# theteamatx/x-edr-trajectory-planning

Measured on AMD Instinct MI355X. Metric: time-optimal path timings/s (7-DOF, 2000 s-samples), 1/2/4/8 MI355X + %HBM roofline, higher is better.
Workload: dtype f64

## Files before the change

x-edr-trajectory-planning_amd/csrc/tpamd_capi.hip:

```cpp
#include "../../include/tpamd.h"

#include <hip/hip_runtime.h>

#include <algorithm>
#include <cmath>
#include <cstdio>
#include <cstdlib>
#include <cstring>
#include <mutex>
#include <new>
#include <vector>

#include "tpamd_kernels.h"
#include "tpamd_launch.h"
#include "tpamd_planner_set.h"
#include "tpamd_readout.h"
#include "tpamd_rescale.h"
#include "tpamd_buffer.h"
#include "tpamd_stop.h"
#include "tpamd_switch.h"
#include "tpamd_fit.h"
#include "tpamd_pose_fit.h"
#include "tpamd_sweep_joint.h"

// ... 181 lines not shown
  Lane lanes[kMaxLanes];
  hipEvent_t ev_fork = nullptr;
  bool in_lane = false;
  hipEvent_t front_wait = nullptr, front_record = nullptr;
  int phase = 0;
  std::vector<hipEvent_t> back_wait;
  int max_lanes = 4;
  int chain_fronts = 2;
  bool order_ragged = true;
  int k1_tpb = 0;
  int k1_tpb_ragged = 64;
  int front_delay_us = 10;
  std::vector<EventPair> events;
  std::vector<EventPair> pool;
  double acc_ms[KI_COUNT] = {};
  int acc_n[KI_COUNT] = {};
};

namespace {

size_t carve_workspace(char *base, int B, int N, int C, Workspace *ws) {
  Stage s(base);
  const size_t nb = (size_t)B, ns = (size_t)B * N;
  Workspace w{};
  w.ds = s.take<double>(nb);
  w.s_start = s.take<double>(nb);
  w.s_end = s.take<double>(nb);
  w.sd_start = s.take<double>(nb);
  w.sdd_start = s.take<double>(nb);
  w.t_start = s.take<double>(nb);
  w.delta = s.take<double>(nb);
  w.err_bits = s.take<uint32_t>(nb);
  w.lim = s.take<double>(nb * 2 * C);
  w.q12 = s.take<double>((ns + kTileSamples) * (C + 2));
  w.m0 = s.take<double>(ns);
  w.z0 = s.take<double>(ns);
  w.X0 = s.take<double>(ns);
  w.Y0 = s.take<double>(ns);
  w.Xz = s.take<double>(ns);
  w.Yz = s.take<double>(ns);
  w.at0 = s.take<uint8_t>(ns);
  w.fix_flag = s.take<uint8_t>(ns);
  w.fix_val = s.take<double>(ns);
  w.m = s.take<double>(ns);
  w.X = s.take<double>(ns);
  w.Y = s.take<double>(ns);
  w.type = s.take<uint8_t>(ns);
  w.sd2 = s.take<double>(ns);
  w.diag = s.take<long long>(nb * kDiagRow);
  w.order = s.take<int32_t>(nb);
  if (ws) *ws = w;
  return s.off;
}

int ensure_workspace(tpamd_engine *e, int B, int N, int C) {
  const size_t need = carve_workspace(nullptr, B, N, C, nullptr);
  if (need > e->ws_buf.bytes) {
    if (e->ws_buf.reserve(need)) return TPAMD_E_HIP;
#ifdef TPAMD_K1_STUDY
    HIPCHK(hipMemset(e->ws_buf.p, 0, need));
#endif
  }
  carve_workspace((char *)e->ws_buf.p, B, N, C, &e->ws);
  e->ws.keep_boundary = e->keep_boundary ? 1 : 0;
#ifdef TPAMD_K1_STUDY
  {
    static void *g_study = nullptr;
// ... 697 lines not shown
    return TPAMD_E_INVALID_ARGUMENT;
  return 0;
}

int cartesian_args(const tpamd_cartesian_batch *bt, const tpamd_cartesian_inputs *in,
                   const tpamd_path_outputs *out) {
  const int D = bt->num_dofs, N = bt->num_samples;
  if (D < 1 || D > 16 || N < 3 || N > 8192) return TPAMD_E_UNSUPPORTED;
  if (!in->ik_positions || !in->jacobians || !in->max_velocity || !in->max_acceleration ||
      !in->max_translational_velocity || !in->max_rotational_velocity || !in->path_start ||
      !in->delta || !in->sd_start || !in->time_start || !out->time || !out->s || !out->sd ||
      !out->sdd || !out->status)
    return TPAMD_E_INVALID_ARGUMENT;
  return 0;
}

int solve_cartesian(tpamd_engine *e, const tpamd_cartesian_batch *bt, const tpamd_cartesian_inputs *in,
                    const tpamd_path_outputs *out, void *hip_stream, const PlanParams *plan, int table_stride) {
  if (!e || !bt || !in || !out) return TPAMD_E_INVALID_ARGUMENT;
  const int B = bt->num_paths, D = bt->num_dofs, N = bt->num_samples;
  if (B <= 0) return B == 0 ? 0 : TPAMD_E_INVALID_ARGUMENT;
  if (int rc = cartesian_args(bt, in, out)) return rc;
  TPAMD_ON_DEVICE(e);
  hipStream_t st = (hipStream_t)hip_stream;
  const int C = 2 * D + 2;
  const int max_loops = bt->max_solver_loops > 0 ? bt->max_solver_loops : 0;
  const bool fused = (D == 6 || D == 7) && !e->force_generic;
  const int stride = plan ? table_stride : N;
  const int *first = plan ? plan->first : nullptr;
  const unsigned gb = (unsigned)((B + 127) / 128);
  PlanParams pp{};
  if (plan) {
    pp = *plan;
    pp.rec_stride = fused ? C + 2 : 2 * D + 2;
  }
  SlotGuard slot_guard(e, st);
  int rc = ensure_workspace(e, B, N, C);
  if (rc) return rc;
  e->last_B = B; e->last_N = N; e->last_time = out->time;
  e->ws.ns = nullptr;
  e->ws.order = nullptr;
  e->ws.amax = in->max_acceleration;
  {
    Timer t(e, st, KI_SETUP);
    hipLaunchKernelGGL(k_setup_cartesian, dim3((B + 127) / 128), dim3(128), 0, st, B, N, D,
                       bt->constraint_safety, in->max_velocity, in->max_acceleration,
                       in->max_translational_velocity, in->max_rotational_velocity,
                       in->path_start, in->delta, in->sd_start, in->sdd_start, in->time_start,
                       e->ws);
    if (plan) hipLaunchKernelGGL(k_plan_mark_skipped, dim3(gb), dim3(128), 0, st, pp, e->ws);
  }
  if (fused) {
    const Workspace &ws = e->ws;
    {
      Timer t(e, st, KI_SAMPLE_LP);
      const int tpb = 256;
      const size_t lds = (2 * (size_t)C + (2 * (size_t)D + 2) * tpb) * 8;
      const dim3 grid((N + tpb - 1) / tpb, B);
      if (D == 6)
        hipLaunchKernelGGL((k_cartesian_lp<1, 6>), grid, dim3(tpb), lds, st, N, in->ik_positions,
                           in->jacobians, ws, stride, first);
      else
        hipLaunchKernelGGL((k_cartesian_lp<1, 7>), grid, dim3(tpb), lds, st, N, in->ik_positions,
                           in->jacobians, ws, stride, first);
      if (plan) hipLaunchKernelGGL(k_plan_project, dim3(gb), dim3(128), 0, st, pp, ws);
    }
    JointSource src;
// ... 2994 lines not shown
```

x-edr-trajectory-planning_amd/csrc/tpamd_kernels.h:

```cpp
#pragma once

#include "tpamd_device.h"
#include "tpamd_cartesian_window.h"
#include "tpamd_quat.h"

namespace tpamd {

constexpr int kDiagExt = 16;
constexpr int kDiagRow = 64 + 2 * kDiagExt;

struct Workspace {
  double *ds, *s_start, *s_end, *sd_start, *sdd_start, *t_start, *delta;
  uint32_t *err_bits;
  const int32_t *ns;
  const double *amax;
  const int32_t *order;
  double *lim;
  double *q12;
  double *m0, *z0, *X0, *Y0, *Xz, *Yz;
  uint8_t *at0;
  uint8_t *fix_flag;
  double *fix_val;
  double *m, *X, *Y;
  uint8_t *type;
// ... 19 lines not shown
  const int tid = threadIdx.x;
  const int shift = (N > 8192) ? 5 : 3;
  hist[tid] = 0;
  __syncthreads();
  for (int b = tid; b < B; b += 1024) {
    const int n = min(max(ns[b], 0), N);
    atomicAdd(&hist[min((N - n) >> shift, kOrderBins - 1)], 1);
  }
  __syncthreads();
  scan[tid] = hist[tid];
  __syncthreads();
  for (int off = 1; off < kOrderBins; off <<= 1) {
    const int v = (tid >= off) ? scan[tid - off] : 0;
    __syncthreads();
    scan[tid] += v;
    __syncthreads();
  }
  hist[tid] = scan[tid] - hist[tid];
  __syncthreads();
  for (int b = tid; b < B; b += 1024) {
    const int n = min(max(ns[b], 0), N);
    order[atomicAdd(&hist[min((N - n) >> shift, kOrderBins - 1)], 1)] = b;
  }
}

struct JointSource {
  const double *q12;
  const double *lim;
  int D;
  int E = 0;
  __device__ __forceinline__ int rows() const { return 2 * D + E; }
  __device__ __forceinline__ int b_only_from() const { return D; }
  static constexpr bool kJoint = true;
  __device__ __forceinline__ int stride() const { return 2 * D + E + 2; }
  __device__ __forceinline__ JointRowsAt at(int b, int N, int idx) const {
    JointRowsAt r;
    r.q12 = q12 + ((size_t)b * N + idx) * stride();
    r.lim_lo = lim + (size_t)b * 2 * rows();
    r.lim_hi = r.lim_lo + rows();
    r.D = D;
    r.E = E;
    return r;
  }
};

struct GenericSource {
  const double *A, *B, *LO, *HI;
  int C;
  __device__ __forceinline__ int rows() const { return C; }
  __device__ __forceinline__ int b_only_from() const { return -1; }
  static constexpr bool kJoint = false;
  __device__ __forceinline__ GlobalRowsAt at(int b, int N, int idx) const {
    const size_t o = ((size_t)b * N + idx) * C;
    GlobalRowsAt r;
    r.A = A + o; r.B = B + o; r.LO = LO + o; r.HI = HI + o;
    return r;
  }
};

static __global__ void k_setup_joint(int B, int N, int D, double safety, const double *vmax,
                              const double *amax, const double *path_start,
                              const double *delta, const double *sd_start,
                              const double *sdd_start, const double *t_start, Workspace ws) {
  const int b = blockIdx.x * blockDim.x + threadIdx.x;
  if (b >= B) return;
  const int C = 2 * D;
  double *lo = ws.lim + (size_t)b * 2 * C, *hi = lo + C;
// ... 140 lines not shown
  if (!live) {
  } else if (parameter < kend + delta) {
    double u = parameter;
    if (u < k0) u = k0;
    if (kend < u) u = kend;
    const int span = knot_span_deg2(s_knots, Kb, u);
    double ders[3][3];
    basis_ders_deg2(s_knots, span, u, ders);
    const double *p0 = s_cp + (size_t)(span - 2) * D, *p1 = p0 + D, *p2 = p1 + D;
#pragma unroll
    for (int d = 0; d < D; d++) {
      double v0 = 0.0, v1 = 0.0, v2 = 0.0;
      v0 += ders[0][0] * p0[d]; v0 += ders[0][1] * p1[d]; v0 += ders[0][2] * p2[d];
      v1 += ders[1][0] * p0[d]; v1 += ders[1][1] * p1[d]; v1 += ders[1][2] * p2[d];
      v2 += ders[2][0] * p0[d]; v2 += ders[2][1] * p1[d]; v2 += ders[2][2] * p2[d];
      if (q_out) q_out[o * D + d] = v0;
      Q1[d * TPB] = v1;
      Q2[d * TPB] = v2;
      if (DT) { q1r[d] = v1; q2r[d] = v2; }
    }
  } else {
    const double *pl = s_cp + (size_t)(Pb - 1) * D;
#pragma unroll
    for (int d = 0; d < D; d++) {
      if (q_out) q_out[o * D + d] = pl[d];
      Q1[d * TPB] = 0.0;
      Q2[d * TPB] = 0.0;
      if (DT) { q1r[d] = 0.0; q2r[d] = 0.0; }
    }
  }
  __syncthreads();
  {
    const int nvalid = min(TPB, Nb - i0);
    double2 *recs = reinterpret_cast<double2 *>(ws.q12 + ((size_t)b * N + i0) * (C + 2));
    const int pairs = D + 1;
    for (int c = tid; c < nvalid * pairs; c += TPB) {
      const int sm = c / pairs, pr = c - sm * pairs;
      recs[c] = (pr < D) ? make_double2(s_Q1[pr * TPB + sm], s_Q2[pr * TPB + sm]) : make_double2(0.0, 0.0);
    }
  }
  if (!live) return;
  LdsRowsJoint r;
  r.Q1 = Q1; r.Q2 = Q2; r.lim_lo = s_lo; r.lim_hi = s_hi; r.stride = TPB; r.D = D;
  if (DT) {
    double sd2max, sddmax, sd2zero, x0, y0;
    lp_find_max_sd2<WORDS, LdsRowsJoint, DT, 2 * DT>(r, C, &sd2max, &sddmax, &sd2zero, D,
                                                     q1r, q2r);
    find_sdd_both_joint_screened<(DT ? DT : 1)>(q1r, q2r, Q1, Q2, TPB, s_hi, sd2max, &x0, &y0);
    ws.m0[o] = sd2max;
    ws.z0[o] = sd2zero;
    ws.X0[o] = x0;
    ws.Y0[o] = y0;
    ws.at0[o] = fabs(sd2max - sd2zero) < kTiny;
  } else {
    boundary_point<WORDS, true>(r, C, o, ws);
  }
#ifdef TPAMD_K1_STUDY
  __syncthreads();
  if (threadIdx.x == 0) {
    unsigned long long t;
    asm volatile("s_memrealtime %0\n\ts_waitcnt lgkmcnt(0)" : "=s"(t)::"memory");
    reinterpret_cast<unsigned long long *>(ws.diag)[2 * (blockIdx.y * gridDim.x + blockIdx.x) + 1] = t;
  }
#endif
}

#ifdef TPAMD_K1_STUDY
#define TPAMD_K1_STUDY_REGS __attribute__((amdgpu_waves_per_eu(5, 5)))
#else
#define TPAMD_K1_STUDY_REGS
#endif
// ... 72 lines not shown
  double ders[3][3];
  basis_ders_deg2(s_knots, span, parameter, ders);
  const double b0 = ders[0][0], b1 = ders[0][1], b2 = ders[0][2];
  const double *t0 = s_t + 3 * (span - 2);
  for (int d = 0; d < 3; d++) {
    double v = 0.0;
    v += b0 * t0[d]; v += b1 * t0[3 + d]; v += b2 * t0[6 + d];
    out[d] = v;
  }
  const double cum1 = b2, cum0 = cum1 + b1;
  const double *r0 = s_r + 4 * (span - 2);
  const Quat p0 = {r0[0], r0[1], r0[2], r0[3]}, p1 = {r0[4], r0[5], r0[6], r0[7]},
             p2 = {r0[8], r0[9], r0[10], r0[11]};
  Quat q = p0;
  q = quat_mul(q, quat_power(quat_mul(quat_inverse(p0), p1), cum0));
  q = quat_mul(q, quat_power(quat_mul(quat_inverse(p1), p2), cum1));
  quat_normalize_positive_real(q);
  out[3] = q.w; out[4] = q.x; out[5] = q.y; out[6] = q.z;
}

static __global__ void k_cartesian_rows(int N, int D, double safety, const double *q_g,
                                 const double *J_g, const double *vmax, const double *amax,
                                 const double *vtrans, const double *vrot, double *A,
                                 double *Bm, double *LO, double *HI, Workspace ws, int table_stride,
                                 const int *first) {
  const int b = blockIdx.y;
  const int i = blockIdx.x * blockDim.x + threadIdx.x;
  if (i >= N) return;
  if (first && (ws.err_bits[b] & kErrSkip)) return;
  const int C = 2 * D + 2;
  const size_t o = (size_t)b * N + i;
  const size_t row = (size_t)b * table_stride + (first ? first[b] : 0) + i;
  cw_rows_at(i, N, D, 1.0 / ws.delta[b], q_g + row * D, J_g + row * 6 * D, vmax + (size_t)b * D,
             amax + (size_t)b * D, safety, vtrans[b], vrot[b], ws.q12 + o * (2 * D + 2), A + o * C, Bm + o * C,
             LO + o * C, HI + o * C);
}

static __global__ void k_setup_cartesian(int B, int N, int D, double safety, const double *vmax,
                                  const double *amax, const double *vtrans, const double *vrot,
                                  const double *path_start, const double *delta,
                                  const double *sd_start, const double *sdd_start,
                                  const double *t_start, Workspace ws) {
  const int b = blockIdx.x * blockDim.x + threadIdx.x;
  if (b >= B) return;
  const int C = 2 * D + 2;
  double *lo = ws.lim + (size_t)b * 2 * C, *hi = lo + C;
  for (int d = 0; d < D; d++) {
    const double am = amax[(size_t)b * D + d] * safety;
    const double vm = vmax[(size_t)b * D + d] * safety;
    hi[d] = am;          lo[d] = -am;
    hi[D + d] = vm * vm; lo[D + d] = 0.0;
  }
  const double vt = vtrans[b], vr = vrot[b];
  hi[2 * D] = vt * vt;     lo[2 * D] = -(vt * vt);
  hi[2 * D + 1] = vr * vr; lo[2 * D + 1] = -(vr * vr);
  double maxw = -DBL_MAX;
  bool lower_ge_upper = false;
  for (int c = 0; c < C; c++) {
    const double w = hi[c] - lo[c];
    if (w > maxw) maxw = w;
    if (lo[c] >= hi[c]) lower_ge_upper = true;
  }
  const double s0 = path_start[b];
  const double s1 = s0 + delta[b] * (N - 1);
  uint32_t bits = 0;
  if (maxw <= 0) bits |= kErrInfeasible;
  if (s0 >= s1) bits |= kErrSRange;
// ... 57 lines not shown
        const double2 *J2 = reinterpret_cast<const double2 *>(Jr);
        double2 jj[D / 2 ? D / 2 : 1];
#pragma unroll
        for (int h = 0; h < D / 2; h++) jj[h] = J2[h];
#pragma unroll
        for (int h = 0; h < D / 2; h++) {
          acc += jj[h].x * s_Q1[(2 * h) * TPB + sm];
          acc += jj[h].y * s_Q1[(2 * h + 1) * TPB + sm];
        }
      } else {
        double jj[D];
#pragma unroll
        for (int d = 0; d < D; d++) jj[d] = Jr[d];
#pragma unroll
        for (int d = 0; d < D; d++) acc += jj[d] * s_Q1[d * TPB + sm];
      }
      V6[r * TPB + sm] = acc;
    }
  }
  __syncthreads();
  double v6[6];
#pragma unroll
  for (int r = 0; r < 6; r++) v6[r] = s_Q2[r * TPB + tid];
  __syncthreads();
#pragma unroll
  for (int d = 0; d < D; d++) Q2[d * TPB] = q2r[d];
  const double bt = (v6[0] * v6[0] + v6[1] * v6[1]) + v6[2] * v6[2];
  const double br = (v6[3] * v6[3] + v6[4] * v6[4]) + v6[5] * v6[5];
  X[0] = bt;
  X[TPB] = br;
  __syncthreads();
  {
    const int nvalid = min(TPB, N - i0);
    double2 *recs = reinterpret_cast<double2 *>(ws.q12 + ((size_t)b * N + i0) * (C + 2));
    constexpr int pairs = D + 2;
    for (int c = tid; c < nvalid * pairs; c += TPB) {
      const int sm = c / pairs, pr = c - sm * pairs;
      double2 v = make_double2(0.0, 0.0);
      if (pr < D) v = make_double2(s_Q1[pr * TPB + sm], s_Q2[pr * TPB + sm]);
      else if (pr == D) v = make_double2(s_X[sm], s_X[TPB + sm]);
      recs[c] = v;
    }
  }
  if (!live) return;
  LdsRowsJoint r;
  r.Q1 = Q1; r.Q2 = Q2; r.lim_lo = s_lo; r.lim_hi = s_hi; r.stride = TPB; r.D = D;
  r.E = 2; r.X = X;
  double sd2max, sddmax, sd2zero, x0 = 0.0, y0 = 0.0;
  lp_find_max_sd2<WORDS, LdsRowsJoint, D, 2 * D + 2>(r, C, &sd2max, &sddmax, &sd2zero, D,
                                                     q1r, q2r);
  {
    const double vt = bt * sd2max, vr = br * sd2max;
    const bool ok = !(vt + kTiny < s_lo[2 * D] || vt - kTiny > s_hi[2 * D]) &&
                    !(vr + kTiny < s_lo[2 * D + 1] || vr - kTiny > s_hi[2 * D + 1]);
    if (ok) find_sdd_both_joint_screened<D>(q1r, q2r, Q1, Q2, TPB, s_hi, sd2max, &x0, &y0);
  }
  ws.m0[o] = sd2max;
  ws.z0[o] = sd2zero;
  ws.X0[o] = x0;
  ws.Y0[o] = y0;
  ws.at0[o] = fabs(sd2max - sd2zero) < kTiny;
}

template <int WORDS>
__global__ void k_lp_rows(int N, int C, const double *Ag, const double *Bg, const double *LOg,
                          const double *HIg, Workspace ws) {
  extern __shared__ double lds[];
  const int TPB = blockDim.x;
  const int tid = threadIdx.x;
  const int b = blockIdx.y;
  double *s_A = lds, *s_B = s_A + (size_t)C * TPB, *s_LO = s_B + (size_t)C * TPB,
         *s_HI = s_LO + (size_t)C * TPB;
  const int i0 = blockIdx.x * TPB;
  const int nvalid = min(TPB, path_samples(ws, b, N) - i0);
// ... 712 lines not shown
    if (icrit < 0 || icrit >= N) icrit = (int)(0.5 * (icrit_lo + icrit_hi));
    if (icrit > 0 && icrit < N - 1) S.put_sd2(icrit, S.m[icrit]);
    if (icrit < 1) { status = 10; break; }
    if (S.m[icrit - 1] <= S.m[icrit]) {
      iback_hi = icrit - 1;
      S.put_sd2(icrit - 1, S.m[icrit - 1]);
    } else {
      iback_hi = icrit;
    }
    iback_lo = S.add_backward(iback_hi);
    iforw_lo = icrit;
    iforw_hi = S.add_forward(iforw_lo);
    if (iback_lo > icrit_lo) { status = 7; break; }
    icrit_lo = iforw_hi;
  }
  __syncthreads();
  sweep_tail(src, ws, b, N, stride, lane, status, lds, lds + N, true, t_out, s_out,
             sd_out, sdd_out, lei_out, dtmax_out, status_out);
}

static __global__ void k_epilogue(int B, int N, int D, const double *rec, const double *sd,
                           const double *sdd, const double *amax, const int32_t *status,
                           const int32_t *ns, double *qd, double *qdd) {
  const size_t e = (size_t)blockIdx.x * blockDim.x + threadIdx.x;
  const size_t total = (size_t)B * N * D;
  if (e >= total) return;
  const size_t o = e / D;
  const int d = (int)(e - o * D);
  const int b = (int)(o / N);
  if (status[b] != 0) return;
  if (ns && (int)(o - (size_t)b * N) >= ns[b]) return;
  const double v = sd[o], a = sdd[o];
  const double v2 = v * v;
  const double2 pr = *reinterpret_cast<const double2 *>(rec + o * (2 * D + 2) + 2 * d);
  const double am = amax[(size_t)b * D + d];
  if (qd) qd[e] = pr.x * v;
  if (qdd) {
    double acc = pr.x * a + pr.y * v2;
    if (acc < -am) acc = -am;
    if (acc > am) acc = am;
    qdd[e] = acc;
  }
}


struct PlanParams {
  int B, N, D, K, cap, max_iterations;
  double max_initial_velocity_error;
  const double *knots;
  const int *np;
  const double *delta;
  const double *initial_velocity;
  const long long *start_ns, *horizon_ns;
  int *path_state;
  int *count;
  double *h_time, *h_s, *h_sd, *h_sdd;
  double *h_q, *h_qd, *h_qdd;
  int *planned_to_end;
  double *path_horizon;
  long long *final_decel_start_ns;
  int *active, *old_state, *offset, *loop, *append, *windows, *status;
  long long *loop_start_ns;
  int *num_active;
  double *path_start, *sd_start, *time_start;
  const double *w_time, *w_s, *w_sd, *w_sdd, *w_q, *w_qd, *w_qdd;
  const int *w_status, *w_lei;
  const double *path_end;
// ... 41 lines not shown
    if (!cw_window(p.path_start[b], p.path_horizon[b], p.delta[b], p.N, p.rows[b], &first, &last)) {
      int need_first, need_count;
      if (p.suspended && cw_window_need(p.path_start[b], p.path_horizon[b], p.delta[b], p.N, p.rows[b], &first, &last,
                                        &need_first, &need_count) == kCwNeedsRows) {
        p.status[b] = kPlanNeedsRows;
        p.suspended[b] = 1;
        p.need_first[b] = need_first;
        p.need_count[b] = need_count;
        p.active[b] = 0;
        return;
      }
      p.status[b] = kPlanInternal;
      p.active[b] = 0;
      return;
    }
    p.first[b] = first;
  }
  p.path_state[b] = 3;
}

static __global__ void k_plan_mark_skipped(PlanParams p, Workspace ws) {
  const int b = blockIdx.x * blockDim.x + threadIdx.x;
  if (b >= p.B) return;
  if (!p.active[b]) ws.err_bits[b] |= kErrSkip;
}

static __global__ void k_plan_project(PlanParams p, Workspace ws) {
  const int b = blockIdx.x * blockDim.x + threadIdx.x;
  if (b >= p.B) return;
  if (!p.active[b]) return;
  const int old_state = p.old_state[b];
  if (old_state != 1 && old_state != 2) return;
  const int D = p.D;
  const double *rec0 = ws.q12 + (size_t)b * p.N * (p.rec_stride ? p.rec_stride : 2 * D + 2);
  const double *iv = p.initial_velocity + (size_t)b * D;
  double nrm2 = 0.0;
  for (int d = 0; d < D; d++) nrm2 += rec0[2 * d] * rec0[2 * d];
  double v = p.sd_start[b];
  if (nrm2 > 100 * DBL_EPSILON) {
    double dot = 0.0;
    for (int d = 0; d < D; d++) dot += iv[d] * rec0[2 * d];
    const double q = dot / nrm2;
    v = (q > 0.0) ? q : 0.0;
  }
  double max_err = 0.0;
  for (int d = 0; d < D; d++) {
    const double e = fabs(rec0[2 * d] * v - iv[d]);
    if (e > max_err) max_err = e;
  }
  if (max_err > p.max_initial_velocity_error) {
    p.status[b] = kPlanInvalidArgument;
    p.active[b] = 0;
    ws.err_bits[b] |= kErrSkip;
    return;
  }
  p.sd_start[b] = v;
  ws.sd_start[b] = v;
}

static __global__ void k_plan_end(PlanParams p) {
  const int b = blockIdx.x * blockDim.x + threadIdx.x;
  if (b >= p.B) return;
  p.append[b] = 0;
  if (!p.active[b]) return;
  const int st = p.w_status[b];
  if (st != 0) { p.status[b] = kPlanInternal; p.active[b] = 0; return; }
  p.append[b] = 1;
// ... 18 lines not shown
static __global__ void k_plan_append(PlanParams p) {
  const int b = blockIdx.y;
  const int i = blockIdx.x * blockDim.x + threadIdx.x;
  if (i >= p.N || !p.append[b]) return;
  const int N = p.N, D = p.D;
  const size_t src = (size_t)b * N + i;
  const size_t dst = (size_t)b * p.cap + p.offset[b] + i;
  if (p.offset[b] + N > p.cap) return;
  p.h_time[dst] = p.w_time[src];
  p.h_s[dst] = p.w_s[src];
  p.h_sd[dst] = p.w_sd[src];
  p.h_sdd[dst] = p.w_sdd[src];
  for (int d = 0; d < D; d++) {
    p.h_q[dst * D + d] = p.w_q[src * D + d];
    p.h_qd[dst * D + d] = p.w_qd[src * D + d];
    p.h_qdd[dst * D + d] = p.w_qdd[src * D + d];
  }
  if (i == 0) p.count[b] = p.offset[b] + N;
}

static __global__ void k_gather_window_q(int N, int D, const double *table_q, int table_stride, const int *first,
                                         const int *active, double *w_q) {
  const int b = blockIdx.y;
  const int e = blockIdx.x * blockDim.x + threadIdx.x;
  if (e >= N * D || !active[b]) return;
  w_q[(size_t)b * N * D + e] = table_q[((size_t)b * table_stride + first[b]) * D + e];
}

static __global__ void k_unpack_records(int B, int N, int D, const double *rec, double *q1, double *q2) {
  const size_t e = (size_t)blockIdx.x * blockDim.x + threadIdx.x;
  if (e >= (size_t)B * N * D) return;
  const size_t o = e / D;
  const int d = (int)(e - o * D);
  const double *r = rec + o * (2 * D + 2) + 2 * d;
  q1[e] = r[0];
  q2[e] = r[1];
}

static __global__ void k_query(int B, int N, int K, const double *time, const double *s,
                        const double *sd, const double *sd2_g, const int32_t *status,
                        const double *tq, double *os, double *osd, double *osdd,
                        int32_t *ok) {
  const size_t o = (size_t)blockIdx.x * blockDim.x + threadIdx.x;
  if (o >= (size_t)B * K) return;
  const int b = (int)(o / K);
  if (status && status[b] != 0) {
    if (ok) ok[o] = 0;
    return;
  }
  const double *tm = time + (size_t)b * N, *sp = s + (size_t)b * N, *sdp = sd + (size_t)b * N,
               *sd2 = sd2_g + (size_t)b * N;
  const double s_start = sp[0], s_end = sp[N - 1];
  const double ds_ = (s_end - s_start) / (N - 1);
  const double inv_ds = 1.0 / ds_;
  const double t = tq[o];
  int good = 1;
  double rs, rsd, rsdd;
  if (t <= tm[0]) {
    rs = s_start; rsd = sdp[0]; rsdd = 0.5 * inv_ds * (sd2[1] - sd2[0]);
  } else if (t >= tm[N - 1]) {
    rs = s_end; rsd = sdp[N - 1]; rsdd = 0.0;
  } else {
    int lo = 0, hi = N - 1;
    while (hi - lo > 1) {
      const int mid = (lo + hi) >> 1;
      if (tm[mid] <= t) lo = mid; else hi = mid;
    }
// ... 166 lines not shown
```

x-edr-trajectory-planning_amd/csrc/tpamd_sweep_joint.h:

```cpp
#pragma once

#include <type_traits>

#include "tpamd_kernels.h"

namespace tpamd {

__device__ __forceinline__ double uniform_f64(double v) {
  const int lo = __builtin_amdgcn_readfirstlane(__double2loint(v));
  const int hi = __builtin_amdgcn_readfirstlane(__double2hiint(v));
  return __hiloint2double(hi, lo);
}
__device__ __forceinline__ double readlane_f64(double v, int lane) {
  const int lo = __builtin_amdgcn_readlane(__double2loint(v), lane);
  const int hi = __builtin_amdgcn_readlane(__double2hiint(v), lane);
  return __hiloint2double(hi, lo);
}
__device__ __forceinline__ int uniform_i32(int v) { return __builtin_amdgcn_readfirstlane(v); }
__device__ __forceinline__ int lds_word(const int *p) {
  return *(const volatile __attribute__((address_space(3))) int *)p;
}

template <int CTRL>
__device__ __forceinline__ double dpp_f64(double v) {
// ... 170 lines not shown
struct RegPack<0> {
  template <int LIMIT> __device__ __forceinline__ void load(const f64x2 *, int) {}
  template <int LIMIT> __device__ __forceinline__ void store(f64x2 *, int) const {}
};

template <int D>
struct JointLayout {
  static constexpr int PARTS = (D <= 7) ? 4 : ((D <= 16) ? 2 : 1);
  static constexpr int RPL = (D + PARTS - 1) / PARTS;
  static constexpr int kCandLanes = 2 * D * PARTS;
  static constexpr int kRows16 = (kCandLanes + 15) / 16;
  static_assert(kCandLanes <= 64, "candidate lanes must fit one wave");
#ifndef TPAMD_CHAIN_STEPS
#define TPAMD_CHAIN_STEPS 16
#endif
  static constexpr int kChain = TPAMD_CHAIN_STEPS;
  static constexpr int GRP = 64 / kChain;
  static constexpr int CPL = (2 * D + GRP - 1) / GRP;
  static constexpr int VPL = (D + GRP - 1) / GRP;
  static constexpr unsigned long long kPart0 =
      (GRP == 4) ? 0x1111111111111111ull : ((GRP == 2) ? 0x5555555555555555ull : ~0ull);
  static_assert(GRP == 1 || GRP == 2 || GRP == 4, "chain steps must be 16, 32 or 64");
};

template <bool MAX>
__device__ __forceinline__ double ext2(double a, double b) {
  return ext2_raw<MAX>(a, b);
}

template <int D, int E = 0>
struct JointSweep {
  typedef JointLayout<D> L;
  static_assert(E == 0 || E == 2, "extra rows come as one pair");
  static constexpr int R = 2 * D + E + 2;
  static constexpr int kMt = D + E / 2;
  static constexpr int kTile = TileCfg<D>::kSamples;
  static constexpr int kChunks = kTile * R / 2;
  static constexpr int kChunksPerLane = (kChunks + 63) / 64;
#ifdef TPAMD_DIAG
  long long diag[32];
  mutable long long diagx[kDiagExt];
#endif
  int N, lane;
  double ds, two_ds;
  double *sd2;
  double *tiles;
  const uint8_t *typel;
  double *sdd_g;
  const double *m_g;
  const double *rec;
  int tag0, tag1;
  double *qd_g, *qdd_g;
  const double *aml;
  uint32_t *dirty;
  int end_idx;
  double lim;
  double chk_hi[L::RPL];
  double vel_hi;
  double vel_lo;
  int vel_mode;
  double ex_hi[E ? E : 1];
  int own_off;
  int chk_off[L::RPL];
  int vel_off;
  double row_lo, row_hi;
  double v_lim[L::CPL];
  int v_off[L::CPL];
  double vv_hi[L::VPL];
  double va_hi[L::VPL];
  int vv_off[L::VPL];

  struct Rows {
    f64x2 own;
    f64x2 chk[L::RPL];
    f64x2 vel;
  };

  static __device__ __forceinline__ void wave_lds_sync() {
    __builtin_amdgcn_fence(__ATOMIC_ACQ_REL, "wavefront");
    __builtin_amdgcn_wave_barrier();
  }

  struct Prefetch {
    RegPack<kChunksPerLane> r;
    double m;
    int tag;
  };
  __device__ __forceinline__ void issue_tile_loads(int t, Prefetch &pf) const {
    const f64x2 *src = reinterpret_cast<const f64x2 *>(rec + (size_t)t * kTile * R);
    pf.r.template load<kChunks>(src, lane);
    pf.m = m_g[min(t * kTile + (lane & (kTile - 1)), N - 1)];
    pf.tag = t;
  }
  __device__ __forceinline__ void store_tile(int slot, const Prefetch &pf) const {
    f64x2 *dst = reinterpret_cast<f64x2 *>(tiles + (size_t)slot * kTile * R);
    pf.r.template store<kChunks>(dst, lane);
    wave_lds_sync();
    if (lane < kTile) {
      const int i = min(pf.tag * kTile + lane, N - 1);
      f64x2 mt;
      mt.x = pf.m;
      mt.y = __longlong_as_double((long long)typel[i]);
      dst[(size_t)lane * (R / 2) + kMt] = mt;
    }
    wave_lds_sync();
  }
  __device__ __forceinline__ void fill_tile(int t, int dir, Prefetch &pf) {
    TPAMD_T0(tf_);
    TPAMD_CNT(27);
    if (pf.tag != t) issue_tile_loads(t, pf);
    wave_lds_sync();
    store_tile(t & 1, pf);
    if (t & 1) tag1 = t; else tag0 = t;
    const int tn = t + dir;
    pf.tag = -1;
    if (tn >= 0 && tn * kTile < N) issue_tile_loads(tn, pf);
    TPAMD_ACC(28, tf_);
  }
  __device__ __forceinline__ void ensure_tile(int idx, int dir, Prefetch &pf) {
    const int t = idx / kTile;
    const int tag = (t & 1) ? tag1 : tag0;
    if (tag != t) fill_tile(t, dir, pf);
  }
  __device__ __forceinline__ const f64x2 *record(int idx) const {
    return reinterpret_cast<const f64x2 *>(tiles) + (size_t)(idx & (2 * kTile - 1)) * (R / 2);
  }
  __device__ __forceinline__ void load_rows(int idx, Rows &r) const {
    const f64x2 *p = record(idx);
    r.own = p[own_off];
#pragma unroll
    for (int k = 0; k < L::RPL; k++) r.chk[k] = p[chk_off[k]];
    r.vel = p[vel_off];
  }
  __device__ __forceinline__ void load_mt(int idx, double &m, int &t) const {
    const f64x2 v = record(idx)[kMt];
    m = v.x;
    t = __double2loint(v.y);
  }

  __device__ __forceinline__ void put_sd2(int i, double v) {
    if (lane == 0) sd2[i] = v;
    __builtin_amdgcn_wave_barrier();
  }
  __device__ __forceinline__ void put_sdd(int i, double v) {
    if (lane == 0) sdd_g[i] = v;
  }

  __device__ __forceinline__ bool emitting() const { return qd_g != nullptr || qdd_g != nullptr; }
  template <bool QD, bool QDD>
  __device__ __forceinline__ void emit_pair(size_t o, f64x2 pr, double v, double a, double amx) const {
    if (QD) qd_g[o] = pr.x * v;
    if (QDD) {
      const double v2 = v * v;
      double acc = pr.x * a + pr.y * v2;
      if (acc < -amx) acc = -amx;
      if (acc > amx) acc = amx;
      qdd_g[o] = acc;
    }
  }
  __device__ __forceinline__ void emit_value(int i, int d, f64x2 pr, double v, double a,
                                             double amx) const {
    const size_t o = (size_t)i * D + d;
    if (qd_g) emit_pair<true, false>(o, pr, v, a, amx);
    if (qdd_g) emit_pair<false, true>(o, pr, v, a, amx);
  }
  __device__ __forceinline__ int emit_range(int lo, int hi, int wv, int nwv, const int *stop = nullptr,
                                            int stop_value = 0) const {
    if (qd_g != nullptr && qdd_g != nullptr) return emit_trips<true, true>(lo, hi, wv, nwv, stop, stop_value);
// ... 298 lines not shown
      } else {
        if (idx < N - 1) sddtmp = sd2[idx + 1] / ds; else sddtmp = 0.0;
      }
    }
    TPAMD_PAIR_WAIT();
    put_sd2(nidx, sd2tmp);
    put_sdd(idx, sddtmp);
    if (!more) end_idx = nidx;
    TPAMD_PAIR_SIGNAL();
    if (!more) return FWD ? N - 1 : 0;
    c.idx = nidx;
    c.cur = sd2tmp;
    c.m_i = m_n;
    c.t_i = c.t_n;
    c.m_n = uniform_f64(m_nn);
    c.t_n = uniform_i32(t_nn);
    c.nxt = uniform_f64(nxt_nn);
    return kContinue;
#undef TPAMD_PAIR_SIGNAL
#undef TPAMD_PAIR_WAIT
  }

  template <bool FWD>
  __device__ __forceinline__ int follow_boundary(Carry &c) {
    constexpr int dir = FWD ? 1 : -1;
    const int j = c.idx + dir * lane;
    const bool in_loop = FWD ? (j < N - 2) : (j > 1);
    bool elig = false;
    double m_jn = 0.0, m_j = 0.0;
    const int jn = j + dir;
    const int tj = max(j, 0) / kTile, tjn = max(jn, 0) / kTile;
    const bool resident = (tj == tag0 || tj == tag1) && (tjn == tag0 || tjn == tag1);
    if (in_loop && j >= 0 && j < N && resident) {
      const f64x2 mt_j = record(j)[kMt], mt_n = record(jn)[kMt];
      m_j = mt_j.x;
      m_jn = mt_n.x;
      const double nxt = sd2[jn];
      elig = (__double2loint(mt_j.y) & kBndTrajectory) && (__double2loint(mt_n.y) & kBndTrajectory) &&
             !(!isnan(nxt) && (nxt < m_jn)) && !(m_jn < 0);
    }
    const unsigned long long mask = __ballot(elig);
    const int L = (~mask == 0ull) ? 64 : (__ffsll((long long)~mask) - 1);
    if (L == 0) return 0;
    const double cur_k = (lane == 0) ? c.cur : m_j;
    const double sddv = FWD ? 0.5 * (m_jn - cur_k) / ds : 0.5 * (cur_k - m_jn) / ds;
    if (lane < L) {
      sd2[j + dir] = m_jn;
      sdd_g[j] = sddv;
    }
    wave_lds_sync();
    c.idx += dir * L;
    c.cur = readlane_f64(m_jn, L - 1);
    return L;
  }

  template <bool FWD>
  __device__ __forceinline__ int follow_chain(Carry &c, Prefetch &pf, int &next_win, bool &curve) {
    constexpr int dir = FWD ? 1 : -1;
    constexpr int K = L::kChain;
    next_win = -1;
    curve = false;
    const int wl = c.win;
    const int r = (wl / L::PARTS) >> 1;
    const double alim = readlane_f64(lim, wl);
    const int j0 = c.idx;
    int jl = j0 + dir * K;
    jl = FWD ? min(jl, N - 1) : max(jl, 0);
    ensure_tile(j0, dir, pf);
    ensure_tile(jl, dir, pf);
    constexpr int G = L::GRP;
    const int k = lane / G;
    int j = j0 + dir * k;
    const bool in_loop = FWD ? (j < N - 2) : (j > 1);
    j = min(max(j, 0), N - 1);
    const int jn = min(max(j + dir, 0), N - 1);
    const f64x2 arow = record(j)[r];
    const double hi_r = readlane_f64(row_hi, r);
    ChainOperands ops;
    load_chain_operands(j, ops);
    const f64x2 mt_j = record(j)[kMt], mt_n = record(jn)[kMt];
    const double nxt = sd2[jn];
    double y = __builtin_amdgcn_rcp(arow.x);
    {
      double e = __builtin_fma(-arow.x, y, 1.0);
      y = __builtin_fma(y, e, y);
      e = __builtin_fma(-arow.x, y, 1.0);
      y = __builtin_fma(y, e, y);
    }
    static_assert(G == 4 && K == 16, "the lane pipeline below assumes four lanes per step and 16-lane DPP rows");
    double x = c.cur, y_out = 0.0;
#pragma unroll
    for (int s = 0; s < K; s++) {
      const double n = alim - arow.y * x;
      const double q0 = n * y;
      const double rem = __builtin_fma(-arow.x, q0, n);
      const double q = __builtin_fma(rem, y, q0);
      y_out = FWD ? x + two_ds * q : x - two_ds * q;
      if (s + 1 < K) {
        int lo = __double2loint(x), hi = __double2hiint(x);
        const int ylo = __double2loint(y_out), yhi = __double2hiint(y_out);
        lo = __builtin_amdgcn_update_dpp(lo, ylo, 0x114, 0xf, 0xf, false);
        hi = __builtin_amdgcn_update_dpp(hi, yhi, 0x114, 0xf, 0xf, false);
        if ((s & 3) == 3) {
          lo = __builtin_amdgcn_update_dpp(lo, ylo, 0x142, 0xe, 0x1, false);
          hi = __builtin_amdgcn_update_dpp(hi, yhi, 0x142, 0xe, 0x1, false);
        }
        x = __hiloint2double(hi, lo);
      }
    }
    const double my_cur = x;
    const double my_sdd = (alim - arow.y * my_cur) / arow.x;
    const double my_new = FWD ? my_cur + two_ds * my_sdd : my_cur - two_ds * my_sdd;
    const double chain_next = y_out;
// ... 258 lines not shown
#endif
};

constexpr int kRefitCap = 128;
constexpr int kRefitLdsBytes = kRefitCap * (4 + 8 + 8);

template <int D, int E>
struct PathBoundary {
  const JointSource &src;
  const Workspace &ws;
  int b, N, stride, lane;
  size_t pb;
  double ds, z00;
  const uint8_t *at_l;
  uint8_t *ff_l, *typel;
  bool keep;
  int *l_idx;
  double *l_val, *l_nxt;
  int count;

  __device__ __forceinline__ void append(bool need, int j, double val, double nxt) {
    const unsigned long long mask = __ballot(need);
    if (!mask) return;
    if (need) {
      const int pos = count + __popcll(mask & ((1ull << lane) - 1ull));
      l_idx[pos] = j;
      l_val[pos] = val;
      l_nxt[pos] = nxt;
    }
    count += __popcll(mask);
  }

  __device__ __forceinline__ void refit_one(int j, double sd2v, double *x, double *y) const {
    constexpr int R = 2 * D + E + 2;
    const f64x2 *rec2 = reinterpret_cast<const f64x2 *>(src.q12 + ((size_t)b * stride + j) * R);
    const double *lim_lo = src.lim + (size_t)b * 2 * (2 * D + E), *lim_hi = lim_lo + 2 * D + E;
    double a[D], bq[D];
#pragma unroll
    for (int d = 0; d < D; d++) {
      const f64x2 p = rec2[d];
      a[d] = p.x;
      bq[d] = p.y;
    }
    bool ok = true;
    if (E > 0) {
      const f64x2 ex = rec2[D];
      const double vt = ex.x * sd2v, vr = ex.y * sd2v;
      ok = !(vt + kTiny < lim_lo[2 * D] || vt - kTiny > lim_hi[2 * D]) &&
           !(vr + kTiny < lim_lo[2 * D + 1] || vr - kTiny > lim_hi[2 * D + 1]);
    }
    if (ok) find_sdd_both_joint_fixed<D>(a, bq, lim_hi, sd2v, x, y);
  }

  __device__ __forceinline__ void finalize(int j, double m, double X, double Y, double m_next) const {
    uint8_t type = kBndNone;
    if (j >= 1 && j <= N - 2) {
      const double sd2p = (m_next - m) / ds;
      const double sd2p_min = 2 * Y;
      const double sd2p_max = 2 * X;
      if (sd2p < sd2p_min) type = kBndSink;
      else if (sd2p > sd2p_max) type = kBndSource;
      if ((sd2p <= sd2p_max) && (sd2p >= sd2p_min)) type = kBndTrajectory;
    }
    if (m == z00) type |= kBndEqualsZ00;
    ws.m[pb + j] = m;
    typel[j] = type;
    if (keep) {
// ... 367 lines not shown
          else refit = true;
        } else if (f_self) {
          m = fvc[u];
          refit = true;
        } else if (iso_n) {
          m = z0c[u]; X = Xzc[u]; Y = Yzc[u];
        } else if (iso_p) {
          m = z0c[u]; X = Xzc[u]; Y = Xzc[u];
        } else {
          m = m0c[u]; X = X0c[u]; Y = Y0c[u];
        }
        const int jn = j + 1;
        if (jn <= N - 1) {
          if (jn + 1 <= N - 2 && ff_l[jn + 1]) m_next = z0n[u];
          else if (ff_l[jn]) m_next = fvn[u];
          else if (ff_l[jn - 1]) m_next = z0n[u];
          else if (iso_at(at_l, N, jn + 1) || iso_at(at_l, N, jn - 1)) m_next = z0n[u];
          else m_next = m0n[u];
        }
        if (!refit) P.finalize(j, m, X, Y, m_next);
      }
      if (P.count + 64 > kRefitCap) P.template flush<true>(diag);
      P.append(refit, j, m, m_next);
    }
  }
  P.template flush<true>(diag);
  __threadfence_block();
  __syncthreads();
  TPAMD_ACCC(22, tp0);
}

template <int D, int E = 0>
struct SweepLds {
  static constexpr int R = 2 * D + E + 2;
  static constexpr int kRingDoubles = 2 * 2 * TileCfg<D>::kSamples * R;
  __host__ __device__ static constexpr int n2(int N) { return (N + 1) & ~1; }
  __host__ __device__ static constexpr int words(int N) { return ((N + 31) / 32 + 1) & ~1; }
  __host__ __device__ static constexpr int type_bytes(int N) { return ((N + 15) / 16) * 16; }
  __host__ __device__ static constexpr size_t bytes(int N) {
    return (size_t)n2(N) * 8 + (size_t)kRingDoubles * 8 + type_bytes(N) + 64 +
           2 * (size_t)words(N) * 4 + 16 * 8 + 32;
  }
};
template <int D, int E = 0>
__host__ __device__ inline size_t sweep_joint_lds_bytes(int N) {
  return SweepLds<D, E>::bytes(N);
}

#ifndef TPAMD_SWEEP_WAVES_PER_EU
#define TPAMD_SWEEP_WAVES_PER_EU 2
#endif
#ifndef TPAMD_SWEEP_WAVES_PER_EU_WIDE
#define TPAMD_SWEEP_WAVES_PER_EU_WIDE 1
#endif
#define TPAMD_SWEEP_OCCUPANCY                                                                          \
  __attribute__((amdgpu_waves_per_eu((D > 8) ? TPAMD_SWEEP_WAVES_PER_EU_WIDE : TPAMD_SWEEP_WAVES_PER_EU, \
                                     (D > 8) ? TPAMD_SWEEP_WAVES_PER_EU_WIDE : TPAMD_SWEEP_WAVES_PER_EU)))
#ifdef TPAMD_K1_STUDY
#define TPAMD_SWEEP_STUDY_REGS __attribute__((amdgpu_num_vgpr(200)))
#else
#define TPAMD_SWEEP_STUDY_REGS
#endif
template <int D, int E = 0>
__global__ void __launch_bounds__(128) TPAMD_SWEEP_OCCUPANCY TPAMD_SWEEP_STUDY_REGS
k_sweep_joint(int stride, int max_loops, JointSource src, Workspace ws, double *t_out, double *s_out,
              double *sd_out, double *sdd_out, int32_t *lei_out, double *dtmax_out,
              int32_t *status_out, double *qd_out, double *qdd_out) {
  extern __shared__ double lds[];
// ... 1 lines not shown
  typedef SweepLds<D, E> LL;
  const int b = uniform_i32(path_of_block(ws, blockIdx.x));
  const int lane = threadIdx.x & 63;
  const int N = path_samples(ws, b, stride);
  const int w = uniform_i32((int)(threadIdx.x >> 6));
  const int tid = threadIdx.x;
  const size_t pb = (size_t)b * stride;
  const uint32_t bits = ws.err_bits[b];
  if (bits & kErrSkip) return;
  if (bits) {
    if (tid == 0) {
      status_out[b] = status_from_bits(bits);
      if (lei_out) lei_out[b] = 0;
      if (dtmax_out) dtmax_out[b] = -1.0;
    }
    return;
  }
#ifdef TPAMD_K1_STUDY
  unsigned long long *study = reinterpret_cast<unsigned long long *>(ws.diag) + 40960 + ((ws.keep_boundary >> 1) & 1) * 4096;
  if (tid == 0) {
    unsigned long long t;
    asm volatile("s_memrealtime %0\n\ts_waitcnt lgkmcnt(0)" : "=s"(t)::"memory");
    unsigned xcc;
    asm volatile("s_getreg_b32 %0, hwreg(HW_REG_XCC_ID)" : "=s"(xcc));
    study[2 * b] = t | ((unsigned long long)(xcc & 15u) << 60);
  }
#endif
  JS S;
  S.N = N; S.lane = lane;
  S.ds = ws.ds[b];
  S.two_ds = 2.0 * S.ds;
  S.sd2 = lds;
  double *ring = lds + LL::n2(N);
  S.tiles = ring + (size_t)w * 2 * JS::kTile * JS::R;
  uint8_t *typel = reinterpret_cast<uint8_t *>(ring + LL::kRingDoubles);
  S.typel = typel;
  int *xchg = reinterpret_cast<int *>(typel + LL::type_bytes(N));
  const int nw = LL::words(N);
  uint32_t *dirty = reinterpret_cast<uint32_t *>(xchg + 16);
  uint32_t *zero = dirty + nw;
  double *aml = reinterpret_cast<double *>(zero + nw);
  double *red = aml + 16;
  S.dirty = dirty;
  S.aml = aml;
  S.sdd_g = sdd_out + pb;
  S.m_g = ws.m + pb;
  S.rec = src.q12 + pb * JS::R;
  S.qd_g = qd_out ? qd_out + pb * D : nullptr;
  S.qdd_g = qdd_out ? qdd_out + pb * D : nullptr;
  S.end_idx = 0;
  S.tag0 = -1; S.tag1 = -1;
  double *sd2 = S.sd2;
  const double sd_start = ws.sd_start[b];
#ifdef TPAMD_DIAG
  long long(&diag)[32] = S.diag;
  long long(&diagx)[kDiagExt] = S.diagx;
  for (int k = 0; k < 32; k++) diag[k] = 0;
  for (int k = 0; k < kDiagExt; k++) diagx[k] = 0;
  volatile long long *fw_stamp = reinterpret_cast<volatile long long *>(red + 2);
#define TPAMD_DIAG_PTR S.diag
#else
#define TPAMD_DIAG_PTR nullptr
#endif
  boundary_passes_for_path<D, E>(src, ws, b, N, stride, tid, reinterpret_cast<uint8_t *>(sd2),
                           reinterpret_cast<uint8_t *>(sd2) + LL::type_bytes(N),
                           reinterpret_cast<char *>(ring), typel, (ws.keep_boundary & 1) != 0,
                           TPAMD_DIAG_PTR);
// ... 541 lines not shown
```

Measured before the change: 2.123 million.

## Drop padding pair from q12 records and move m/type into separate LDS ring

```diff
diff --git a/x-edr-trajectory-planning_amd/csrc/tpamd_capi.hip b/x-edr-trajectory-planning_amd/csrc/tpamd_capi.hip
--- a/x-edr-trajectory-planning_amd/csrc/tpamd_capi.hip
+++ b/x-edr-trajectory-planning_amd/csrc/tpamd_capi.hip
@@ -237,7 +237,7 @@
   w.delta = s.take<double>(nb);
   w.err_bits = s.take<uint32_t>(nb);
   w.lim = s.take<double>(nb * 2 * C);
-  w.q12 = s.take<double>((ns + kTileSamples) * (C + 2));
+  w.q12 = s.take<double>((ns + kTileSamples) * C);
   w.m0 = s.take<double>(ns);
   w.z0 = s.take<double>(ns);
   w.X0 = s.take<double>(ns);
@@ -1001,7 +1001,7 @@
   PlanParams pp{};
   if (plan) {
     pp = *plan;
-    pp.rec_stride = fused ? C + 2 : 2 * D + 2;
+    pp.rec_stride = fused ? C : 2 * D;
   }
   SlotGuard slot_guard(e, st);
   int rc = ensure_workspace(e, B, N, C);
diff --git a/x-edr-trajectory-planning_amd/csrc/tpamd_kernels.h b/x-edr-trajectory-planning_amd/csrc/tpamd_kernels.h
--- a/x-edr-trajectory-planning_amd/csrc/tpamd_kernels.h
+++ b/x-edr-trajectory-planning_amd/csrc/tpamd_kernels.h
@@ -75,7 +75,7 @@
   __device__ __forceinline__ int rows() const { return 2 * D + E; }
   __device__ __forceinline__ int b_only_from() const { return D; }
   static constexpr bool kJoint = true;
-  __device__ __forceinline__ int stride() const { return 2 * D + E + 2; }
+  __device__ __forceinline__ int stride() const { return 2 * D + E; }
   __device__ __forceinline__ JointRowsAt at(int b, int N, int idx) const {
     JointRowsAt r;
     r.q12 = q12 + ((size_t)b * N + idx) * stride();
@@ -282,11 +282,11 @@
   __syncthreads();
   {
     const int nvalid = min(TPB, Nb - i0);
-    double2 *recs = reinterpret_cast<double2 *>(ws.q12 + ((size_t)b * N + i0) * (C + 2));
-    const int pairs = D + 1;
+    double2 *recs = reinterpret_cast<double2 *>(ws.q12 + ((size_t)b * N + i0) * C);
+    const int pairs = D;
     for (int c = tid; c < nvalid * pairs; c += TPB) {
       const int sm = c / pairs, pr = c - sm * pairs;
-      recs[c] = (pr < D) ? make_double2(s_Q1[pr * TPB + sm], s_Q2[pr * TPB + sm]) : make_double2(0.0, 0.0);
+      recs[c] = make_double2(s_Q1[pr * TPB + sm], s_Q2[pr * TPB + sm]);
     }
   }
   if (!live) return;
@@ -425,7 +425,7 @@
   const size_t o = (size_t)b * N + i;
   const size_t row = (size_t)b * table_stride + (first ? first[b] : 0) + i;
   cw_rows_at(i, N, D, 1.0 / ws.delta[b], q_g + row * D, J_g + row * 6 * D, vmax + (size_t)b * D,
-             amax + (size_t)b * D, safety, vtrans[b], vrot[b], ws.q12 + o * (2 * D + 2), A + o * C, Bm + o * C,
+             amax + (size_t)b * D, safety, vtrans[b], vrot[b], ws.q12 + o * (2 * D), A + o * C, Bm + o * C,
              LO + o * C, HI + o * C);
 }
 
@@ -549,14 +549,12 @@
   __syncthreads();
   {
     const int nvalid = min(TPB, N - i0);
-    double2 *recs = reinterpret_cast<double2 *>(ws.q12 + ((size_t)b * N + i0) * (C + 2));
-    constexpr int pairs = D + 2;
+    double2 *recs = reinterpret_cast<double2 *>(ws.q12 + ((size_t)b * N + i0) * C);
+    constexpr int pairs = D + 1;
     for (int c = tid; c < nvalid * pairs; c += TPB) {
       const int sm = c / pairs, pr = c - sm * pairs;
-      double2 v = make_double2(0.0, 0.0);
-      if (pr < D) v = make_double2(s_Q1[pr * TPB + sm], s_Q2[pr * TPB + sm]);
-      else if (pr == D) v = make_double2(s_X[sm], s_X[TPB + sm]);
-      recs[c] = v;
+      recs[c] = (pr < D) ? make_double2(s_Q1[pr * TPB + sm], s_Q2[pr * TPB + sm])
+                         : make_double2(s_X[sm], s_X[TPB + sm]);
     }
   }
   if (!live) return;
@@ -1335,7 +1333,7 @@
   if (ns && (int)(o - (size_t)b * N) >= ns[b]) return;
   const double v = sd[o], a = sdd[o];
   const double v2 = v * v;
-  const double2 pr = *reinterpret_cast<const double2 *>(rec + o * (2 * D + 2) + 2 * d);
+  const double2 pr = *reinterpret_cast<const double2 *>(rec + o * (2 * D) + 2 * d);
   const double am = amax[(size_t)b * D + d];
   if (qd) qd[e] = pr.x * v;
   if (qdd) {
@@ -1443,7 +1441,7 @@
   const int old_state = p.old_state[b];
   if (old_state != 1 && old_state != 2) return;
   const int D = p.D;
-  const double *rec0 = ws.q12 + (size_t)b * p.N * (p.rec_stride ? p.rec_stride : 2 * D + 2);
+  const double *rec0 = ws.q12 + (size_t)b * p.N * (p.rec_stride ? p.rec_stride : 2 * D);
   const double *iv = p.initial_velocity + (size_t)b * D;
   double nrm2 = 0.0;
   for (int d = 0; d < D; d++) nrm2 += rec0[2 * d] * rec0[2 * d];
@@ -1528,7 +1526,7 @@
   if (e >= (size_t)B * N * D) return;
   const size_t o = e / D;
   const int d = (int)(e - o * D);
-  const double *r = rec + o * (2 * D + 2) + 2 * d;
+  const double *r = rec + o * (2 * D) + 2 * d;
   q1[e] = r[0];
   q2[e] = r[1];
 }
diff --git a/x-edr-trajectory-planning_amd/csrc/tpamd_sweep_joint.h b/x-edr-trajectory-planning_amd/csrc/tpamd_sweep_joint.h
--- a/x-edr-trajectory-planning_amd/csrc/tpamd_sweep_joint.h
+++ b/x-edr-trajectory-planning_amd/csrc/tpamd_sweep_joint.h
@@ -226,8 +226,7 @@
 struct JointSweep {
   typedef JointLayout<D> L;
   static_assert(E == 0 || E == 2, "extra rows come as one pair");
-  static constexpr int R = 2 * D + E + 2;
-  static constexpr int kMt = D + E / 2;
+  static constexpr int R = 2 * D + E;
   static constexpr int kTile = TileCfg<D>::kSamples;
   static constexpr int kChunks = kTile * R / 2;
   static constexpr int kChunksPerLane = (kChunks + 63) / 64;
@@ -289,13 +288,12 @@
   __device__ __forceinline__ void store_tile(int slot, const Prefetch &pf) const {
     f64x2 *dst = reinterpret_cast<f64x2 *>(tiles + (size_t)slot * kTile * R);
     pf.r.template store<kChunks>(dst, lane);
-    wave_lds_sync();
     if (lane < kTile) {
       const int i = min(pf.tag * kTile + lane, N - 1);
       f64x2 mt;
       mt.x = pf.m;
       mt.y = __longlong_as_double((long long)typel[i]);
-      dst[(size_t)lane * (R / 2) + kMt] = mt;
+      mt_ring()[slot * kTile + lane] = mt;
     }
     wave_lds_sync();
   }
@@ -319,6 +317,10 @@
   __device__ __forceinline__ const f64x2 *record(int idx) const {
     return reinterpret_cast<const f64x2 *>(tiles) + (size_t)(idx & (2 * kTile - 1)) * (R / 2);
   }
+  __device__ __forceinline__ f64x2 *mt_ring() const {
+    return reinterpret_cast<f64x2 *>(tiles) + 2 * kTile * (R / 2);
+  }
+  __device__ __forceinline__ f64x2 mt_at(int idx) const { return mt_ring()[idx & (2 * kTile - 1)]; }
   __device__ __forceinline__ void load_rows(int idx, Rows &r) const {
     const f64x2 *p = record(idx);
     r.own = p[own_off];
@@ -327,7 +329,7 @@
     r.vel = p[vel_off];
   }
   __device__ __forceinline__ void load_mt(int idx, double &m, int &t) const {
-    const f64x2 v = record(idx)[kMt];
+    const f64x2 v = mt_at(idx);
     m = v.x;
     t = __double2loint(v.y);
   }
@@ -692,7 +694,7 @@
     const int tj = max(j, 0) / kTile, tjn = max(jn, 0) / kTile;
     const bool resident = (tj == tag0 || tj == tag1) && (tjn == tag0 || tjn == tag1);
     if (in_loop && j >= 0 && j < N && resident) {
-      const f64x2 mt_j = record(j)[kMt], mt_n = record(jn)[kMt];
+      const f64x2 mt_j = mt_at(j), mt_n = mt_at(jn);
       m_j = mt_j.x;
       m_jn = mt_n.x;
       const double nxt = sd2[jn];
@@ -738,7 +740,7 @@
     const double hi_r = readlane_f64(row_hi, r);
     ChainOperands ops;
     load_chain_operands(j, ops);
-    const f64x2 mt_j = record(j)[kMt], mt_n = record(jn)[kMt];
+    const f64x2 mt_j = mt_at(j), mt_n = mt_at(jn);
     const double nxt = sd2[jn];
     double y = __builtin_amdgcn_rcp(arow.x);
     {
@@ -1063,7 +1065,7 @@
   }
 
   __device__ __forceinline__ void refit_one(int j, double sd2v, double *x, double *y) const {
-    constexpr int R = 2 * D + E + 2;
+    constexpr int R = 2 * D + E;
     const f64x2 *rec2 = reinterpret_cast<const f64x2 *>(src.q12 + ((size_t)b * stride + j) * R);
     const double *lim_lo = src.lim + (size_t)b * 2 * (2 * D + E), *lim_hi = lim_lo + 2 * D + E;
     double a[D], bq[D];
@@ -1497,8 +1499,9 @@
 
 template <int D, int E = 0>
 struct SweepLds {
-  static constexpr int R = 2 * D + E + 2;
-  static constexpr int kRingDoubles = 2 * 2 * TileCfg<D>::kSamples * R;
+  static constexpr int R = 2 * D + E;
+  static constexpr int kWaveDoubles = 2 * TileCfg<D>::kSamples * (R + 2);
+  static constexpr int kRingDoubles = 2 * kWaveDoubles;
   __host__ __device__ static constexpr int n2(int N) { return (N + 1) & ~1; }
   __host__ __device__ static constexpr int words(int N) { return ((N + 31) / 32 + 1) & ~1; }
   __host__ __device__ static constexpr int type_bytes(int N) { return ((N + 15) / 16) * 16; }
@@ -1566,7 +1569,7 @@
   S.two_ds = 2.0 * S.ds;
   S.sd2 = lds;
   double *ring = lds + LL::n2(N);
-  S.tiles = ring + (size_t)w * 2 * JS::kTile * JS::R;
+  S.tiles = ring + (size_t)w * LL::kWaveDoubles;
   uint8_t *typel = reinterpret_cast<uint8_t *>(ring + LL::kRingDoubles);
   S.typel = typel;
   int *xchg = reinterpret_cast<int *>(typel + LL::type_bytes(N));
```

Result: no change. 2.140 million (median of 6 runs) (+0.8%).
